# lightonai/next-plaid

Measured on AMD Instinct MI355X. Metric: queries/sec + p50 latency, k=10, 10M-doc x 300-tok x d128 PLAID index, 1/2/4/8 GPU, higher is better.
Workload: dtype f32 (split-bf16 hi/lo MFMA on the residual term of MaxSim, f32-class accuracy)

## Files before the change

next-plaid_amd/csrc/np_index.hip:

```cpp
#include "np_internal.h"

#include <hipcub/hipcub.hpp>

#include <algorithm>
#include <memory>
#include <thread>
#include <math.h>
#include <stdio.h>
#include <time.h>
#include <stdlib.h>
#include <string.h>

namespace np {

int DevBuf::reserve(size_t bytes) {
  if (bytes <= cap) return NP_OK;
  if (p) (void)hipFree(p);
  p = nullptr;
  cap = 0;
  size_t want = bytes + (bytes >> 3) + 256;
  hipError_t e = hipMalloc(&p, want);
  if (e != hipSuccess) {
    p = nullptr;
    set_error("hipMalloc(%zu bytes) failed: %s", want, hipGetErrorString(e));
// ... 29 lines not shown
  if (o->n_contexts <= 0) o->n_contexts = 2;
  if (o->n_contexts > 16) o->n_contexts = 16;
  if (o->max_batch <= 0) o->max_batch = 64;
  if (o->max_query_tokens <= 0) o->max_query_tokens = 64;
  return NP_OK;
}

bool set_tuning(Tuning* t, const std::string& n, int value) {
  auto clamp = [](int v, int lo, int hi) { return std::min(std::max(v, lo), hi); };
  if (n == "s4_mode") t->s4_mode = clamp(value, 0, 8);
  else if (n == "s4_minb") t->s4_minb = std::max(value, 1);
  else if (n == "s4_nbx") t->s4_nbx = clamp(value, 8, 512);
  else if (n == "s4_swz") t->s4_swz = value != 0;
  else if (n == "s4_filter") t->s4_filter = value != 0;
  else if (n == "s4_hot") t->s4_hot = clamp(value, 0, 500);
  else if (n == "s4_planes") t->s4_planes = value != 0;
  else if (n == "s4_pexp") t->s4_pexp = clamp(value, 5, 40);
  else if (n == "s4_lpd") t->s4_lpd = value == 2 ? 2 : 4;
  else if (n == "s4_qm") t->s4_qm = value != 0;
  else if (n == "s4_pnbx") t->s4_pnbx = clamp(value, 8, 512);
  else if (n == "s3_slices") t->s3_slices = value != 0;
  else if (n == "s4_warm") t->s4_warm = clamp(value, 0, 1000);
  else if (n == "ub_ncut") t->ub_ncut = clamp(value, 1, 512);
  else if (n == "s3_bisect") t->s3_bisect = clamp(value, 0, 1);
  else if (n == "s3_gain") t->s3_gain = clamp(value, 0, 2);
  else if (n == "s3_gain_mult") t->s3_gain_mult = clamp(value, 1, 16);
  else if (n == "s3_gain_direct") t->s3_gain_direct = clamp(value, 0, 64);
  else if (n == "s4_hot_auto") t->s4_hot_auto = clamp(value, 0, 0x7fffffff);
  else if (n == "ub_nt") t->ub_nt = value < 0 || value > 2 ? 0 : value;
  else if (n == "ub_steal") t->ub_steal = value < 1 ? 1 : value;
  else if (n == "ub_nbx") t->ub_nbx = clamp(value, 8, 256);
  else if (n == "ub_direct") t->ub_direct = clamp(value, 0, 16);
#ifdef NP_DIAGNOSTICS
  else if (n == "s4_probe") t->s4_probe = clamp(value, 0, 7);
#endif
  else if (n == "ub_static") t->ub_static = value != 0;
  else if (n == "hot_static") t->hot_static = value != 0;
  else if (n == "s6_xcd") t->s6_xcd = value != 0;
  else if (n == "s6_tiles") t->s6_tiles = value != 0;
  else if (n == "s6_lds") t->s6_lds = clamp(value, 0, 2);
  else if (n == "gemm_cpw") t->gemm_cpw = value == 2 ? 2 : 1;
  else if (n == "s1_split") t->s1_split = value != 0;
  else if (n == "exact_rowmax") t->exact_rowmax = value != 0;
  else return false;
  return true;
}

void read_tuning_env(Tuning* t) {
  static const char* const knobs[][2] = {
      {"NP_S4_MODE", "s4_mode"}, {"NP_S4_MINB", "s4_minb"}, {"NP_S4_NBX", "s4_nbx"}, {"NP_S4_SWZ", "s4_swz"},
      {"NP_S4_FILTER", "s4_filter"}, {"NP_S4_HOT", "s4_hot"}, {"NP_S4_PLANES", "s4_planes"}, {"NP_S4_PEXP", "s4_pexp"}, {"NP_S4_LPD", "s4_lpd"}, {"NP_S4_QM", "s4_qm"}, {"NP_S4_PNBX", "s4_pnbx"}, {"NP_S4_WARM", "s4_warm"}, {"NP_UB_NCUT", "ub_ncut"}, {"NP_S3_BISECT", "s3_bisect"}, {"NP_S3_GAIN", "s3_gain"}, {"NP_S3_GAIN_MULT", "s3_gain_mult"}, {"NP_S3_GAIN_DIRECT", "s3_gain_direct"}, {"NP_S4_HOT_AUTO", "s4_hot_auto"}, {"NP_S3_SLICES", "s3_slices"}, {"NP_UB_NT", "ub_nt"},
      {"NP_UB_STEAL", "ub_steal"}, {"NP_UB_NBX", "ub_nbx"}, {"NP_UB_DIRECT", "ub_direct"}, {"NP_UB_STATIC", "ub_static"}, {"NP_HOT_STATIC", "hot_static"}, {"NP_S6_XCD", "s6_xcd"}, {"NP_S6_TILES", "s6_tiles"}, {"NP_S6_LDS", "s6_lds"}, {"NP_GEMM_CPW", "gemm_cpw"}, {"NP_S1_SPLIT", "s1_split"},
      {"NP_EXACT_ROWMAX", "exact_rowmax"}};
  for (const auto& k : knobs) {
    const char* e = getenv(k[0]);
    if (e && *e) (void)set_tuning(t, k[1], atoi(e));
  }
#ifdef NP_DIAGNOSTICS
  if (const char* e = getenv("NP_S4_PROBE")) (void)set_tuning(t, "s4_probe", atoi(e));
#endif
}

static void default_workspace(DeviceIndex* ix) {
  ix->ws_auto = ix->opts.workspace_bytes <= 0;
  ix->ws_budget = ix->opts.workspace_bytes;
  ix->ws_budget_open = ix->opts.workspace_bytes;
  if (!ix->ws_auto) return;
  size_t free_b = 0, total_b = 0;
  int64_t ws = (int64_t)8 << 30;
  if (hipMemGetInfo(&free_b, &total_b) == hipSuccess) {
    const int64_t share = ((int64_t)free_b - ((int64_t)4 << 30)) / std::max(ix->opts.n_contexts, 1);
    ws = std::min<int64_t>((int64_t)16 << 30, std::max<int64_t>((int64_t)2 << 30, share));
  }
  ix->opts.workspace_bytes = ws;
// ... 1512 lines not shown
```

next-plaid_amd/csrc/np_internal.h:

```cpp
#pragma once
#include <hip/hip_runtime.h>
#include <stdint.h>
#include <algorithm>
#include <atomic>
#include <mutex>
#include <condition_variable>
#include <string>
#include <vector>
#include "../../include/nextplaid_hip.h"

namespace np {

struct CodeArr {
  const void* p;
  int wide;
  __device__ __forceinline__ uint32_t operator[](int64_t i) const {
    return wide ? static_cast<const uint32_t*>(p)[i] : (uint32_t)static_cast<const uint16_t*>(p)[i];
  }
};

void set_error(const char* fmt, ...) __attribute__((format(printf, 1, 2)));
const char* last_error();
void clear_error();

// ... 105 lines not shown
struct DevBuf {
  void* p = nullptr;
  size_t cap = 0;
  int reserve(size_t bytes);
  void release();
  template <class T> T* as() const { return (T*)p; }
};

struct Workspace;

struct Context {
  hipStream_t stream = nullptr;
  hipEvent_t ev[10] = {};
  Workspace* ws = nullptr;
  bool busy = false;
  uint64_t last_use = 0;
};

struct Tuning {
  int s4_mode = 4;
  int s4_minb = 8;
  int s4_nbx = 128;
  int s4_swz = 1;
  int s3_bisect = 1;
  int s3_slices = 1;
  int s3_gain = 1;
  int s3_gain_mult = 3;
  int s3_gain_direct = 16;
  int s4_filter = 1;
  int s4_hot = 60;
  int s4_hot_auto = 200000;
  int s4_planes = 1;
  int s4_lpd = 2;
  int s4_pnbx = 96;
  int s4_qm = 1;
  int s4_pexp = 15;
  int s4_warm = 0;
  int ub_ncut = 96;
  int ub_direct = 8;
  int hot_static = 1;
  int ub_static = 0;
  int s4_probe = 0;
  int ub_nbx = 96;
  int ub_steal = 16384;
  int ub_nt = 2;
  int s6_xcd = 1;
// ... 103 lines not shown
```

next-plaid_amd/csrc/np_kernels.h:

```cpp
#pragma once
#include <hip/hip_runtime.h>
#include <stdint.h>

namespace np {

typedef float f32x16 __attribute__((ext_vector_type(16)));
typedef __bf16 bf16x8 __attribute__((ext_vector_type(8)));

#define NP_NEG_INF (-__builtin_huge_valf())
#define NP_MAX_QT 8

__device__ __forceinline__ uint32_t okey(float x) {
  uint32_t b = __float_as_uint(x);
  uint32_t k = (b & 0x80000000u) ? ~b : (b | 0x80000000u);
  return ((b & 0x7F800000u) == 0x7F800000u) ? 0u : k;
}
__device__ __forceinline__ float unkey(uint32_t k) {
  uint32_t b = (k & 0x80000000u) ? (k ^ 0x80000000u) : ~k;
  return __uint_as_float(b);
}
__device__ __forceinline__ bool finitef(float x) { return (__float_as_uint(x) & 0x7F800000u) != 0x7F800000u; }
__device__ __forceinline__ float readlane_f(float v, int lane) {
  return __int_as_float(__builtin_amdgcn_readlane(__float_as_int(v), lane));
}
// ... 400 lines not shown
  }
}

struct ProbeP {
  const float* QCT;
  const uint32_t* gmax;
  const int32_t* qoff;
  int64_t K, KP;
  int LQP;
  int nprobe;
  const int32_t* nprobe_dev;
  const uint32_t* elig;
  const int32_t* n_elig;
  int has_thr;
  float thr;
  int lds_gm;
  int64_t slab;
  uint32_t* cellbits;
  uint32_t* tauq;
  uint32_t* cells_tmp;
  uint32_t* cells;
  int32_t* n_cells;
  Counters* ctr;
};

#define NP_PROBE_CAPG 64

template <class Pred>
__device__ __forceinline__ uint32_t wave_count(int nslots, const uint32_t (&keys)[32], Pred&& pred) {
  uint32_t mine = 0;
#pragma unroll
  for (int j = 0; j < 32; ++j) mine += (j < nslots && pred(keys[j])) ? 1u : 0u;
  uint32_t cnt = 0;
#pragma unroll
  for (int b = 0; b < 6; ++b) cnt += (uint32_t)__popcll(__ballot((mine >> b) & 1u)) << b;
  return cnt;
}

__device__ __forceinline__ void wave_select_mark(int nslots, uint32_t n_probe, const uint32_t (&keys)[32],
                                                 uint32_t& tau, uint32_t& rem) {
  uint32_t prefix = 0;
  for (int bit = 31; bit >= 0; --bit) {
    const uint32_t trial = prefix | (1u << bit);
    if (wave_count(nslots, keys, [&](uint32_t k) { return k >= trial; }) >= n_probe) prefix = trial;
  }
  const uint32_t gt = wave_count(nslots, keys, [&](uint32_t k) { return k > prefix; });
  tau = prefix;
  rem = n_probe > gt ? n_probe - gt : 0u;
}

template <int QW>
__global__ void __launch_bounds__(256) probe_mark_kernel(ProbeP p) {
  __shared__ uint32_t hist[256 * QW];
  __shared__ uint32_t part[256];
  __shared__ uint32_t s_prefix[QW], s_rem[QW], s_taug[QW], s_gcnt[QW];
  __shared__ uint32_t s_glist[QW * NP_PROBE_CAPG];
  extern __shared__ uint32_t s_gm[];
  constexpr int NR = 256 / QW;
  const bool lds_gm = p.lds_gm != 0;
  const int b = blockIdx.y, qc = blockIdx.x, tid = threadIdx.x, q = tid % QW, r = tid / QW;
  const int wave = tid >> 6, lane = tid & 63;
  const int Lq = p.qoff[b + 1] - p.qoff[b];
  const int64_t G = p.KP >> 5;
  const int LQP = p.LQP;
  const float* QCT = p.QCT + (int64_t)b * p.KP * LQP;
  const uint32_t* gm = p.gmax + (int64_t)b * G * LQP;
  uint32_t* bits = p.cellbits + (int64_t)b * G;
  const int64_t pool = p.elig ? (int64_t)*p.n_elig : p.K;
  const int64_t eff = p.nprobe_dev ? (int64_t)*p.nprobe_dev : (int64_t)p.nprobe;
  const uint32_t n_probe = (uint32_t)min(eff, pool);
  const bool take_all = pool <= (int64_t)n_probe;
  uint32_t* tauq = p.tauq + (int64_t)b * LQP;

  if (n_probe > 0 && take_all && Lq > 0) {
    if (qc != 0) return;
    for (int64_t w = tid; w < G; w += 256) {
      uint32_t m = p.elig ? p.elig[w] : 0xFFFFFFFFu;
      const int64_t c0 = w * 32;
      if (c0 + 32 > p.K) m &= (c0 >= p.K) ? 0u : ((1u << (p.K - c0)) - 1u);
      if (m) atomicOr(&bits[w], m);
    }
  } else if (n_probe > 0) {
    {
      if (qc * QW >= Lq) return;
      const int qq = qc * QW + q;
      const bool qvalid = qq < Lq;
      const bool use_groups = G > (int64_t)n_probe;
      if (lds_gm) {
        for (int64_t g0 = r; g0 < G; g0 += 16 * NR) {
          uint32_t kv[16];
#pragma unroll
          for (int u = 0; u < 16; ++u) kv[u] = (qvalid && g0 + NR * u < G) ? gm[(g0 + NR * u) * LQP + qq] : 0u;
#pragma unroll
          for (int u = 0; u < 16; ++u)
            if (g0 + NR * u < G) s_gm[(g0 + NR * u) * QW + q] = kv[u];
        }
        __syncthreads();
      }
      auto each_group = [&](auto&& cb) {
        if (!qvalid) return;
        if (lds_gm) {
          for (int64_t g = r; g < G; g += NR) cb(g, s_gm[g * QW + q]);
        } else {
          for (int64_t g = r; g < G; g += 8 * NR) {
            uint32_t kv[8];
#pragma unroll
            for (int u = 0; u < 8; ++u) kv[u] = (g + NR * u < G) ? gm[(g + NR * u) * LQP + qq] : 0u;
#pragma unroll
            for (int u = 0; u < 8; ++u)
              if (g + NR * u < G) cb(g + NR * u, kv[u]);
          }
        }
      };
      if (use_groups) {
        radix_select<QW>([&](auto&& cb) { each_group([&](int64_t, uint32_t key) { cb(key); }); }, n_probe, hist, part,
                         s_prefix, s_rem, tid);
        if (r == 0) s_taug[q] = s_prefix[q];
      } else if (r == 0) {
        s_taug[q] = 0;
      }
// ... 462 lines not shown
  int c = 0;
  for (int k = 0; k < NP_CHUNK_WORDS / 256; ++k) {
    const int64_t w = (int64_t)ch * NP_CHUNK_WORDS + k * 256 + threadIdx.x;
    if (w < NW) c += __popc(bits[w]);
  }
#pragma unroll
  for (int o = 32; o > 0; o >>= 1) c += __shfl_xor(c, o);
  if ((threadIdx.x & 63) == 0) atomicAdd(&s_cnt, c);
  __syncthreads();
  if (threadIdx.x == 0) chunk_counts[(int64_t)b * nchunks + ch] = s_cnt;
}

struct RoundPlan {
  int32_t* n_cand;
  int64_t* cand_base;
  int32_t* round_of;
  int32_t* round_tab;
  int32_t* order;
};

__global__ void __launch_bounds__(256) plan_rounds_kernel(const int32_t* __restrict__ chunk_counts, int nchunks, int B,
                                                          int64_t pool, int max_rounds, RoundPlan rp, Counters* ctr,
                                                          const int32_t* __restrict__ n_direct = nullptr ) {
  __shared__ int s_n[256];
  const int tid = threadIdx.x, lane = tid & 63, wave = tid >> 6;
  for (int b = wave; b < B; b += 4) {
    int c = 0;
    if (n_direct) c = lane == 0 ? n_direct[b] : 0;
    else
    for (int j = lane; j < nchunks; j += 64) c += chunk_counts[(int64_t)b * nchunks + j];
#pragma unroll
    for (int o = 32; o > 0; o >>= 1) c += __shfl_xor(c, o);
    if (lane == 0) s_n[b] = c;
  }
  __syncthreads();
  if (tid == 0) {
    int64_t cur = 0;
    unsigned long long total = 0;
    int r = 0;
    for (int i = 0; i < 2 * max_rounds; ++i) rp.round_tab[i] = 0;
    rp.round_tab[0] = 0;
    for (int b = 0; b < B; ++b) {
      const int n = s_n[b];
      if (cur + n > pool && r + 1 < max_rounds) {
        rp.round_tab[2 * r + 1] = b;
        ++r;
        rp.round_tab[2 * r] = b;
        cur = 0;
      }
      rp.n_cand[b] = (cur + n > pool) ? (int)max((int64_t)0, pool - cur) : n;
      rp.cand_base[b] = cur;
      rp.round_of[b] = r;
      cur += rp.n_cand[b];
      total += (unsigned long long)rp.n_cand[b];
    }
    rp.round_tab[2 * r + 1] = B;
    rp.round_tab[2 * max_rounds] = r + 1;
    if (!n_direct) atomicAdd(&ctr->n_candidates, total);
    atomicMax(&ctr->n_rounds, (unsigned long long)(r + 1));
  }
  __syncthreads();
  for (int b = tid; b < B; b += 256) {
    const int r = rp.round_of[b], rb = rp.round_tab[2 * r], re = rp.round_tab[2 * r + 1];
    const int n = rp.n_cand[b];
    int rank = 0;
    for (int j = rb; j < re; ++j) {
      const int nj = rp.n_cand[j];
      rank += (nj > n || (nj == n && j < b)) ? 1 : 0;
    }
    rp.order[rb + rank] = b;
  }
}

template <class Steal>
__device__ __forceinline__ int xcd_next_query(int32_t* slots, int32_t* ticket, int x, int step, int B,
                                              const int32_t* order, int rb, int re, Steal&& steal) {
  if (step > B) return -3;
  int32_t* slot = slots + (int64_t)x * (B + 1) + step;
  int v = __hip_atomic_load(slot, __ATOMIC_RELAXED, __HIP_MEMORY_SCOPE_AGENT);
  if (v == -1 && atomicCAS(slot, -1, -2) == -1) {
    const int t = atomicAdd(ticket, 1) + 1;
    v = (t < re - rb) ? order[rb + t] : steal();
    __hip_atomic_store(slot, v, __ATOMIC_RELAXED, __HIP_MEMORY_SCOPE_AGENT);
    return v;
  }
  while (v == -1 || v == -2) {
    __builtin_amdgcn_s_sleep(4);
    v = __hip_atomic_load(slot, __ATOMIC_RELAXED, __HIP_MEMORY_SCOPE_AGENT);
  }
  return v;
}

// ... 1404 lines not shown
    ndoc += __shfl_xor(ndoc, o);
  }
  __shared__ unsigned long long s_cnt[3];
  __syncthreads();
  if (tid == 0) s_cnt[0] = s_cnt[1] = s_cnt[2] = 0;
  __syncthreads();
  if (lane == 0 && toks) {
    atomicAdd(&s_cnt[0], toks);
    atomicAdd(&s_cnt[1], ucnt);
    atomicAdd(&s_cnt[2], ndoc);
  }
  __syncthreads();
  if (tid == 0 && s_cnt[0] && ctr) {
    if (count_tokens) {
      atomicAdd(&ctr->n_cand_tokens, s_cnt[0]);
      atomicAdd(&ctr->n_cand_dcodes, s_cnt[1]);
    } else {
      atomicAdd(&ctr->n_level2, s_cnt[2]);
    }
    atomicAdd(&ctr->n_cand_codes, s_cnt[1]);
  }
}

__global__ void __launch_bounds__(256) ub_thr_kernel(const uint32_t* __restrict__ hist, int hshift, int slack, int n_sel,
                                                     const int32_t* __restrict__ n_cand, RoundPlan rp, int round,
                                                     const uint32_t* __restrict__ qflag, uint32_t* __restrict__ thr) {
  __shared__ uint32_t s_part[256];
  constexpr int BPT = NP_UB_BINS / 256;
  const int b = blockIdx.x, tid = threadIdx.x;
  if (rp.round_of[b] != round) return;
  if (qflag[b] != 0 || n_cand[b] <= n_sel) {
    if (tid == 0) thr[b] = 0;
    return;
  }
  const uint32_t* hb = hist + (int64_t)b * NP_UB_BINS;
  const int top = (255 - tid) * BPT;
  uint32_t mine = 0;
#pragma unroll
  for (int k4 = 0; k4 < BPT / 4; ++k4) {
    const uint4 v = *reinterpret_cast<const uint4*>(hb + top + 4 * k4);
    mine += v.x + v.y + v.z + v.w;
  }
  s_part[tid] = mine;
  __syncthreads();
  if (tid == 0) {
    uint32_t cum = 0;
    int t = 0;
    for (; t < 255; ++t) {
      if (cum + s_part[t] >= (uint32_t)n_sel) break;
      cum += s_part[t];
    }
    int bin = (255 - t) * BPT + BPT - 1;
    for (; bin > (255 - t) * BPT; --bin) {
      if (cum + hb[bin] >= (uint32_t)n_sel) break;
      cum += hb[bin];
    }
    thr[b] = (uint32_t)max(0, bin - ((slack + (1 << hshift) - 1) >> hshift));
  }
}

struct CutP {
  const uint4* src;
  const int32_t* n_src_a;
  const int32_t* n_src_b;
  const uint16_t* U;
  const uint32_t* lo;
  const uint32_t* hi;
  int zero_mode;
  const uint4* all_src;
  const int32_t* n_all;
  uint4* dst;
  const int32_t* dst_begin;
  int32_t* n_dst;
  int hshift;
  Counters* ctr;
};

__global__ void __launch_bounds__(256) ub_cut_kernel(CutP p, RoundPlan rp, int round) {
  __shared__ int s_wcnt[4], s_base;
  __shared__ unsigned long long s_cnt[2];
  const int b = blockIdx.y, tid = threadIdx.x, lane = tid & 63, wave = tid >> 6;
  if (rp.round_of[b] != round) return;
  const uint32_t lo = p.lo[b], hi = p.hi ? p.hi[b] : 0xFFFFFFFFu;
  const bool all = lo == 0;
  if (all && p.zero_mode == 1) return;
  const uint4* src = all ? p.all_src : p.src;
  const int64_t n = all ? (int64_t)p.n_all[b] : (int64_t)p.n_src_a[b] + (p.n_src_b ? p.n_src_b[b] : 0);
  const int64_t pbase = rp.cand_base[b];
  const int64_t dbase = pbase + (p.dst_begin ? p.dst_begin[b] : 0);
  if (tid == 0) s_cnt[0] = s_cnt[1] = 0;
  unsigned long long toks = 0, ucnt = 0;
  constexpr int PT = 8;
  for (int64_t i0 = (int64_t)blockIdx.x * (256 * PT); i0 < n; i0 += (int64_t)gridDim.x * (256 * PT)) {
    bool keep[PT];
    unsigned long long bal[PT];
    int wtot = 0;
#pragma unroll
    for (int k = 0; k < PT; ++k) {
      const int64_t i = i0 + k * 256 + tid;
      bool kp = i < n;
      if (kp && !all) {
        const uint32_t bin = min((uint32_t)p.U[pbase + i] >> p.hshift, (uint32_t)(NP_UB_BINS - 1));
        kp = bin >= lo && bin < hi;
      }
      keep[k] = kp;
      bal[k] = __ballot(kp);
// ... 2515 lines not shown
```

next-plaid_amd/csrc/np_search.hip:

```cpp
#include "np_internal.h"
#include "np_kernels.h"

#include <algorithm>
#include <array>
#include <cmath>
#include <stdlib.h>
#include <string.h>
#include <type_traits>
#include <utility>

namespace np {

struct Workspace {
  DevBuf q, qoff, Qt, Qb, Qbl, QCT, gmax, tauq, cellbits, cells_tmp, cells, n_cells, docbits, chunk_counts, cand, cand_meta, approx, n_cand,
      cand_base, round_of, round_tab, QCU, qinv, qflag, ub, ub_hist, ub_thr, ub_cursor, q_order, xcd_slots, surv_meta, n_surv, n_list2, sel_keys, sel_doc, nsel, exact, out_ids, out_scores, out_keys, out_counts, ctr, subset,
      subset_bits, elig, misc, cut, cmaxu, chist, ub2, ub_hist2, ub_thr2, list_meta, n_l1, n_l2, qpad, planes, levels, hotbits,
      gain, gsmall, ghist, s0_meta, s0_u, gacc, gdeep;
  void* h_pin = nullptr;
  size_t h_pin_cap = 0;
  unsigned long long* h_gain = nullptr;
  uint64_t h_gain_key = 0;
  hipEvent_t done = nullptr;
  bool done_valid = false;
  static constexpr int NBUF = 66;
  std::array<DevBuf*, NBUF> all_bufs() {
    return {&q, &qoff, &Qt, &Qb, &Qbl, &QCT, &gmax, &tauq, &cellbits, &cells_tmp, &cells, &n_cells, &docbits, &chunk_counts, &cand, &cand_meta, &approx, &n_cand, &cand_base, &round_of, &round_tab, &QCU, &qinv, &qflag, &ub, &ub_hist, &ub_thr, &ub_cursor, &q_order, &xcd_slots, &surv_meta, &n_surv, &n_list2, &sel_keys, &sel_doc, &nsel, &exact, &out_ids, &out_scores, &out_keys, &out_counts, &ctr, &subset, &subset_bits, &elig, &misc, &cut, &cmaxu, &chist, &ub2, &ub_hist2, &ub_thr2, &list_meta, &n_l1, &n_l2, &qpad, &planes, &levels, &hotbits, &gain, &gsmall, &ghist, &s0_meta, &s0_u, &gacc, &gdeep};
  }
  void release_all() {
    for (DevBuf* b : all_bufs()) b->release();
    if (h_pin) (void)hipHostFree(h_pin);
    h_pin = nullptr;
    h_pin_cap = 0;
    if (h_gain) (void)hipHostFree(h_gain);
    h_gain = nullptr;
    if (done) (void)hipEventDestroy(done);
    done = nullptr;
  }
  size_t total_bytes() {
    size_t t = 0;
    for (DevBuf* b : all_bufs()) t += b->cap;
    return t;
  }
  unsigned probe_tick = 0;
  size_t pool_bytes() const {
    return cand.cap + cand_meta.cap + approx.cap + ub.cap + surv_meta.cap + ub2.cap + list_meta.cap;
  }
  void release_pool() {
    DevBuf* pool[] = {&cand, &cand_meta, &approx, &ub, &surv_meta, &ub2, &list_meta};
    for (DevBuf* b : pool) b->release();
// ... 127 lines not shown
    return NP_ERR_INVALID_ARGUMENT;
  }
  return NP_OK;
}

constexpr int NP_POOL_ENTRY = 60;
struct WsPlan {
  int S = 1;
  int64_t pool = 1;
  int max_rounds = 1;
};

static int64_t per_query_bytes(const DeviceIndex* ix, int LQP, int n_sel, int top_k) {
  const int64_t KP = ix->KP, G = KP / 32, NW = (ix->n_docs + 31) / 32;
  const int64_t nchunks = (NW + NP_CHUNK_WORDS - 1) / NP_CHUNK_WORDS;
  return KP * LQP * 6
         + KP + 1024
         + KP * 6 + G * 4 + NP_UB_BINS * 8
         + (ix->d_ivf_split.get() ? (int64_t)ix->n_ranges * NP_GAIN_RANGE : 0)
         + NP_UB_BINS * 8
         + G * LQP * 4 + G * 4
         + KP * 8
         + (int64_t)LQP * 4
         + std::max<int64_t>(NW, 1) * 4
         + std::max<int64_t>(nchunks, 1) * 4
         + (int64_t)ix->dim * LQP * 8
         + (int64_t)std::max(n_sel, 1) * 16 + (int64_t)std::max(top_k, 1) * 20 + 64;
}

static WsPlan plan_workspace(const DeviceIndex* ix, int B, int LQP, const np_search_params* prm, int64_t probed_cells = 0) {
  WsPlan w;
  const int64_t budget = ix->ws_budget.load(std::memory_order_relaxed);
  const int64_t pq = std::max<int64_t>(per_query_bytes(ix, LQP, n_sel_of(prm), prm->top_k), 1);
  const int64_t nd = std::max<int64_t>(ix->n_docs, 1);
  const int cap = (int)std::min<int64_t>(std::min<int64_t>(ix->opts.max_batch, NP_S4_MAXB), std::max(B, 1));
  int64_t S = std::min<int64_t>(cap, std::max<int64_t>(1, (budget * 3 / 4) / pq));
  while (S > 1 && S * pq + 2 * nd * NP_POOL_ENTRY > budget) --S;
  w.S = (int)S;
  int64_t worst_q = nd;
  if (probed_cells > 0 && !ix->ivf_top_prefix.empty())
    worst_q = std::max<int64_t>(1, std::min(nd, ix->ivf_top_prefix[(size_t)std::min<int64_t>(probed_cells, ix->K)]));
  const int64_t worst = S * worst_q;
  int64_t pool = (budget - S * pq) / NP_POOL_ENTRY;
  pool = std::min(worst, std::max(pool, std::min<int64_t>(2, S) * worst_q));
  w.pool = std::max<int64_t>(pool, 1);
  w.max_rounds = (worst <= w.pool) ? 1 : (int)std::min<int64_t>(S, worst / (w.pool - worst_q + 1) + 1);
// ... 356 lines not shown
  if (!ix->gain_run.load(std::memory_order_relaxed)) ix->gain_skip.store(3, std::memory_order_relaxed);
  return true;
}

static void settle_zeroth_level(const DeviceIndex* ix, Workspace& w, const CallState* cs, PassPlan& p) {
  p.gain_path = p.gain_possible && (ix->tune.s3_gain != 1 || gain_level_runs(ix, w, cs, p.B, p.LQP));
  p.gain_deep = p.gain_path && p.deep_wanted;
  if (p.gain_path && cs->prm.has_threshold && !p.gain_deep) p.gain_path = false;
}

static int reserve_pass(const DeviceIndex* ix, const CallState* cs, const PassPlan& p, Workspace& w) {
  const size_t B = (size_t)p.B, KP = (size_t)p.KP, G = (size_t)p.G, LQP = (size_t)p.LQP, dim = (size_t)ix->dim;
  const size_t pool = (size_t)p.pool, RB = (size_t)p.RB;
  const size_t nsel1 = (size_t)std::max(cs->n_sel, 1), topk1 = (size_t)std::max(cs->prm.top_k, 1);
  const size_t nw1 = (size_t)std::max<int64_t>(p.NW, 1);
  if (ix->ldim != ix->dim) NP_TRY(w.qpad.reserve((size_t)std::max<int64_t>(p.rows, 1) * dim * 4));
  NP_TRY(w.Qt.reserve(B * dim * LQP * 4));
  NP_TRY(w.Qb.reserve(B * dim * LQP * 2));
  NP_TRY(w.Qbl.reserve(B * dim * LQP * 2));
  NP_TRY(w.QCT.reserve(B * KP * LQP * 4));
  NP_TRY(w.gmax.reserve(B * G * LQP * 4));
  NP_TRY(w.cellbits.reserve(B * G * 4));
  NP_TRY(w.tauq.reserve(B * LQP * 4));
  NP_TRY(w.cells_tmp.reserve(B * KP * 4));
  NP_TRY(w.cells.reserve(B * KP * 4));
  NP_TRY(w.n_cells.reserve(B * 4));
  NP_TRY(w.docbits.reserve(B * nw1 * 4));
  NP_TRY(w.chunk_counts.reserve(B * (size_t)std::max(p.nchunks, 1) * 4));
  NP_TRY(w.cand.reserve(pool * 4));
  NP_TRY(w.cand_meta.reserve(pool * 16));
  NP_TRY(w.approx.reserve(pool * 4));
  NP_TRY(w.n_cand.reserve(B * 4));
  NP_TRY(w.cand_base.reserve(B * 8));
  NP_TRY(w.round_of.reserve(B * 4));
  NP_TRY(w.round_tab.reserve((size_t)(2 * p.max_rounds + 1) * 4));
  NP_TRY(w.q_order.reserve(B * 4));
  NP_TRY(w.n_list2.reserve(B * 4));
  NP_TRY(w.qinv.reserve(B * 4));
  NP_TRY(w.qflag.reserve(B * 4));
  if (p.use_filter) {
    NP_TRY(w.QCU.reserve(B * KP * RB));
    NP_TRY(w.ub.reserve(pool * 2));
    NP_TRY(w.ub_hist.reserve(B * NP_UB_BINS * 4));
    NP_TRY(w.surv_meta.reserve(pool * 16));
    NP_TRY(w.n_surv.reserve(B * 4));
    NP_TRY(w.ub_thr.reserve(B * 4));
// ... 164 lines not shown
  const np_search_params& prm = cs->prm;
  ProbeP pp;
  pp.QCT = w.QCT.as<float>();
  pp.gmax = w.gmax.as<uint32_t>();
  pp.qoff = d_qoff;
  pp.K = ix->K;
  pp.KP = p.KP;
  pp.LQP = p.LQP;
  pp.nprobe = prm.n_ivf_probe;
  pp.nprobe_dev = p.use_elig ? w.misc.as<int32_t>() + 1 : nullptr;
  pp.elig = p.use_elig ? (cs->elig_global ? cs->elig_global : w.elig.as<uint32_t>()) : nullptr;
  pp.n_elig = p.use_elig ? w.misc.as<int32_t>() : nullptr;
  pp.has_thr = prm.has_threshold;
  pp.thr = prm.centroid_score_threshold;
  pp.slab = p.batched ? (int64_t)prm.centroid_batch_size : 0;
  pp.cellbits = w.cellbits.as<uint32_t>();
  pp.tauq = w.tauq.as<uint32_t>();
  pp.cells_tmp = w.cells_tmp.as<uint32_t>();
  pp.cells = w.cells.as<uint32_t>();
  pp.n_cells = w.n_cells.as<int32_t>();
  pp.ctr = w.ctr.as<Counters>();
  const size_t gm_lds = (size_t)(p.KP / 32) * 4 * 4;
  pp.lds_gm = gm_lds <= 32 * 1024 ? 1 : 0;
  auto probe = [&](const ProbeP& pr) {
    if (pr.lds_gm) probe_mark_kernel<4><<<dim3((unsigned)(p.LQP / 4), B), 256, gm_lds, st>>>(pr);
    else probe_mark_kernel<8><<<dim3((unsigned)(p.LQP / 8), B), 256, 0, st>>>(pr);
    probe_finish_kernel<<<dim3(NP_PROBE_NF, B), 256, 0, st>>>(pr);
  };
  probe(pp);
  if (!p.gain_deep) return;
  const GDeep gd(w.gdeep.p, p);
  ProbeP p2 = pp;
  p2.nprobe = p.gain_depth;
  p2.has_thr = 0;
  p2.cellbits = gd.marks;
  p2.tauq = gd.tauq;
  p2.n_cells = gd.n_cells;
  p2.cells = gd.cells;
  p2.ctr = nullptr;
  probe(p2);
  if (prm.has_threshold)
    cells_to_bits_kernel<<<B, 256, 0, st>>>(w.cells.as<uint32_t>(), w.n_cells.as<int32_t>(), p.KP, gd.kept);
}

RoundPlan Pass::round_plan() const {
  RoundPlan rp;
  rp.n_cand = w.n_cand.as<int32_t>();
  rp.cand_base = w.cand_base.as<int64_t>();
  rp.round_of = w.round_of.as<int32_t>();
  rp.round_tab = w.round_tab.as<int32_t>();
  rp.order = w.q_order.as<int32_t>();
  return rp;
}

int Pass::ub_bounds(const RoundPlan& rpx, int r, int max_rounds, int32_t* sl, uint32_t* cur, const uint4* meta,
                    const int32_t* begin, const int32_t* count, const int32_t* n_all, uint16_t* U, uint32_t* hist,
                    int count_tokens, int direct_wpq, bool floor_rows) const {
// ... 183 lines not shown
    }
  } else if (ix->T > 0) {
    if (matvec) {
      launch_matvec(st, ix, w, d_q, d_qoff, B, w.cand_meta.as<uint4>(), w.n_cand.as<int32_t>(), rp, r);
      count_work_kernel<<<dim3(32, (unsigned)B), 256, 0, st>>>(w.cand_meta.as<uint4>(), w.n_cand.as<int32_t>(), rp, r,
                                                               w.ctr.as<Counters>());
    } else {
      launch_approx(st, ix, w, d_qoff, B, p.LQP, w.cand_meta.as<uint4>(), w.n_cand.as<int32_t>(), rp, r, p.max_rounds,
                    w.ctr.as<Counters>());
    }
  }
  if (cs->timed && r == 0) NP_HIP(hipEventRecord(cs->ctx->ev[4], st));
  if (cs->n_sel > 0) {
    sp.round = r;
    select_kernel<<<B, 1024, (size_t)cs->NSELP * 8, st>>>(sp);
  }
  return NP_OK;
}

int Pass::single_level_cut(int r, const RoundPlan& rp) const {
  const int B = p.B;
  NP_TRY(ub_bounds(rp, r, p.max_rounds, slots((size_t)r * 3), cursor(0), w.cand_meta.as<uint4>(), nullptr, w.n_cand.as<int32_t>(),
                   w.n_cand.as<int32_t>(), w.ub.as<uint16_t>(), w.ub_hist.as<uint32_t>(), 1, 0, false));
  ub_thr_kernel<<<B, 256, 0, st>>>(w.ub_hist.as<uint32_t>(), p.hshift, p.slack, cs->n_sel, w.n_cand.as<int32_t>(), rp, r,
                                   w.qflag.as<uint32_t>(), w.ub_thr.as<uint32_t>());
  CutP cp{};
  cp.hshift = p.hshift;
  cp.all_src = w.cand_meta.as<uint4>();
  cp.n_all = w.n_cand.as<int32_t>();
  cp.src = w.cand_meta.as<uint4>();
  cp.n_src_a = w.n_cand.as<int32_t>();
  cp.U = w.ub.as<uint16_t>();
  cp.lo = w.ub_thr.as<uint32_t>();
  cp.zero_mode = 0;
  cp.dst = w.surv_meta.as<uint4>();
  cp.n_dst = w.n_surv.as<int32_t>();
  cp.ctr = w.ctr.as<Counters>();
  ub_cut_kernel<<<dim3(n_cut(), B), 256, 0, st>>>(cp, rp, r);
  return NP_OK;
}

int Pass::two_level_cut(int r, const RoundPlan& rp) const {
  const int B = p.B;
  const unsigned ncut = n_cut();
  auto ub = [&](int lvl, const int32_t* begin, const int32_t* count, int direct_wpq, bool floor_rows) {
    return ub_bounds(rp, r, p.max_rounds, slots((size_t)r * 3 + lvl), cursor(lvl), w.list_meta.as<uint4>(), begin, count,
                     w.n_cand.as<int32_t>(), w.ub2.as<uint16_t>(), w.ub_hist2.as<uint32_t>(), 0, direct_wpq, floor_rows);
  };
  CutP cp{};
  cp.hshift = p.hshift;
  cp.all_src = w.cand_meta.as<uint4>();
  cp.n_all = w.n_cand.as<int32_t>();
  if (cs->timed && r == 0) NP_HIP(hipEventRecord(cs->ctx->ev[8], st));
  NP_TRY(hot_level(r, rp));
  if (cs->timed && r == 0) {
    NP_HIP(hipEventRecord(cs->ctx->ev[9], st));
    cs->hot_timed = true;
  }
  ub_thr_kernel<<<B, 256, 0, st>>>(w.ub_hist.as<uint32_t>(), p.hshift, 0, cs->n_sel, w.n_cand.as<int32_t>(), rp, r,
                                   w.qflag.as<uint32_t>(), w.ub_thr.as<uint32_t>());
  cp.src = w.cand_meta.as<uint4>();
  cp.n_src_a = w.n_cand.as<int32_t>();
  cp.U = w.ub.as<uint16_t>();
  cp.lo = w.ub_thr.as<uint32_t>();
  cp.zero_mode = 1;
  cp.dst = w.list_meta.as<uint4>();
  cp.n_dst = w.n_l1.as<int32_t>();
  ub_cut_kernel<<<dim3(ncut, B), 256, 0, st>>>(cp, rp, r);
  NP_TRY(ub(1, nullptr, w.n_l1.as<int32_t>(), ix->tune.ub_direct, false));
  ub_thr_kernel<<<B, 256, 0, st>>>(w.ub_hist2.as<uint32_t>(), p.hshift, p.slack, cs->n_sel, w.n_cand.as<int32_t>(), rp, r,
                                   w.qflag.as<uint32_t>(), w.ub_thr2.as<uint32_t>());
  cp.lo = w.ub_thr2.as<uint32_t>();
  cp.hi = w.ub_thr.as<uint32_t>();
  cp.dst_begin = w.n_l1.as<int32_t>();
  cp.n_dst = w.n_l2.as<int32_t>();
  ub_cut_kernel<<<dim3(ncut, B), 256, 0, st>>>(cp, rp, r);
  NP_TRY(ub(2, w.n_l1.as<int32_t>(), w.n_l2.as<int32_t>(), 0, true));
  ub_thr_kernel<<<B, 256, 0, st>>>(w.ub_hist2.as<uint32_t>(), p.hshift, p.slack, cs->n_sel, w.n_cand.as<int32_t>(), rp, r,
                                   w.qflag.as<uint32_t>(), w.ub_thr2.as<uint32_t>());
  cp.src = w.list_meta.as<uint4>();
  cp.n_src_a = w.n_l1.as<int32_t>();
  cp.n_src_b = w.n_l2.as<int32_t>();
  cp.U = w.ub2.as<uint16_t>();
  cp.lo = w.ub_thr2.as<uint32_t>();
  cp.hi = nullptr;
  cp.zero_mode = 0;
  cp.dst = w.surv_meta.as<uint4>();
  cp.dst_begin = nullptr;
  cp.n_dst = w.n_surv.as<int32_t>();
  cp.ctr = w.ctr.as<Counters>();
  ub_cut_kernel<<<dim3(ncut, B), 256, 0, st>>>(cp, rp, r);
  return NP_OK;
}

int Pass::hot_level(int r, const RoundPlan& rp) const {
  const int B = p.B;
  const int64_t KP = p.KP;
  const int old_cap = ix->code_wide ? 64 : 128;
  const int plpd = (ix->ublock_stride > old_cap || ix->tune.s4_lpd == 4) ? 4 : 2;
  const unsigned pnbx = (unsigned)ix->tune.s4_pnbx;
  return with_codes(ix->code_wide, [&](auto ct) -> int {
    using CT = decltype(ct);
// ... 856 lines not shown
```

Measured before the change: 20290.

## Add threshold-first probe list, fuse UB threshold into cut, parallelize round planning

Three separate changes. A new probe_thr_kernel first lists the centroids whose max score clears the query threshold, so the probe marking kernel can rank only those listed cells and fall back to the full group scan when the list overflows. Separately, the ub_thr_kernel launches are removed: each ub_cut_kernel block now computes the histogram threshold itself through a parallel wave scan, and one block writes it out. plan_rounds_kernel is also rewritten to build its round table and ordering from shared-memory arrays in parallel instead of serially through global memory. Together these aim to cut kernel launches and serial work, at the cost of repeating the threshold scan in every cut block and extra complexity in the probe path.

```diff
diff --git a/next-plaid_amd/csrc/np_index.hip b/next-plaid_amd/csrc/np_index.hip
--- a/next-plaid_amd/csrc/np_index.hip
+++ b/next-plaid_amd/csrc/np_index.hip
@@ -75,6 +75,7 @@
   else if (n == "s3_slices") t->s3_slices = value != 0;
   else if (n == "s4_warm") t->s4_warm = clamp(value, 0, 1000);
   else if (n == "ub_ncut") t->ub_ncut = clamp(value, 1, 512);
+  else if (n == "s2_thr_first") t->s2_thr_first = value != 0;
   else if (n == "s3_bisect") t->s3_bisect = clamp(value, 0, 1);
   else if (n == "s3_gain") t->s3_gain = clamp(value, 0, 2);
   else if (n == "s3_gain_mult") t->s3_gain_mult = clamp(value, 1, 16);
@@ -102,7 +103,7 @@
 void read_tuning_env(Tuning* t) {
   static const char* const knobs[][2] = {
       {"NP_S4_MODE", "s4_mode"}, {"NP_S4_MINB", "s4_minb"}, {"NP_S4_NBX", "s4_nbx"}, {"NP_S4_SWZ", "s4_swz"},
-      {"NP_S4_FILTER", "s4_filter"}, {"NP_S4_HOT", "s4_hot"}, {"NP_S4_PLANES", "s4_planes"}, {"NP_S4_PEXP", "s4_pexp"}, {"NP_S4_LPD", "s4_lpd"}, {"NP_S4_QM", "s4_qm"}, {"NP_S4_PNBX", "s4_pnbx"}, {"NP_S4_WARM", "s4_warm"}, {"NP_UB_NCUT", "ub_ncut"}, {"NP_S3_BISECT", "s3_bisect"}, {"NP_S3_GAIN", "s3_gain"}, {"NP_S3_GAIN_MULT", "s3_gain_mult"}, {"NP_S3_GAIN_DIRECT", "s3_gain_direct"}, {"NP_S4_HOT_AUTO", "s4_hot_auto"}, {"NP_S3_SLICES", "s3_slices"}, {"NP_UB_NT", "ub_nt"},
+      {"NP_S4_FILTER", "s4_filter"}, {"NP_S4_HOT", "s4_hot"}, {"NP_S4_PLANES", "s4_planes"}, {"NP_S4_PEXP", "s4_pexp"}, {"NP_S4_LPD", "s4_lpd"}, {"NP_S4_QM", "s4_qm"}, {"NP_S4_PNBX", "s4_pnbx"}, {"NP_S4_WARM", "s4_warm"}, {"NP_UB_NCUT", "ub_ncut"}, {"NP_S3_BISECT", "s3_bisect"}, {"NP_S2_THR_FIRST", "s2_thr_first"}, {"NP_S3_GAIN", "s3_gain"}, {"NP_S3_GAIN_MULT", "s3_gain_mult"}, {"NP_S3_GAIN_DIRECT", "s3_gain_direct"}, {"NP_S4_HOT_AUTO", "s4_hot_auto"}, {"NP_S3_SLICES", "s3_slices"}, {"NP_UB_NT", "ub_nt"},
       {"NP_UB_STEAL", "ub_steal"}, {"NP_UB_NBX", "ub_nbx"}, {"NP_UB_DIRECT", "ub_direct"}, {"NP_UB_STATIC", "ub_static"}, {"NP_HOT_STATIC", "hot_static"}, {"NP_S6_XCD", "s6_xcd"}, {"NP_S6_TILES", "s6_tiles"}, {"NP_S6_LDS", "s6_lds"}, {"NP_GEMM_CPW", "gemm_cpw"}, {"NP_S1_SPLIT", "s1_split"},
       {"NP_EXACT_ROWMAX", "exact_rowmax"}};
   for (const auto& k : knobs) {
diff --git a/next-plaid_amd/csrc/np_internal.h b/next-plaid_amd/csrc/np_internal.h
--- a/next-plaid_amd/csrc/np_internal.h
+++ b/next-plaid_amd/csrc/np_internal.h
@@ -151,6 +151,7 @@
   int s4_minb = 8;
   int s4_nbx = 128;
   int s4_swz = 1;
+  int s2_thr_first = 1;
   int s3_bisect = 1;
   int s3_slices = 1;
   int s3_gain = 1;
diff --git a/next-plaid_amd/csrc/np_kernels.h b/next-plaid_amd/csrc/np_kernels.h
--- a/next-plaid_amd/csrc/np_kernels.h
+++ b/next-plaid_amd/csrc/np_kernels.h
@@ -446,7 +446,83 @@
   uint32_t* cells;
   int32_t* n_cells;
   Counters* ctr;
+  uint32_t* thr_list;
+  const uint32_t* qflag;
 };
+
+#define NP_PROBE_THR_CAP 64
+#define NP_PROBE_THR_OVF 0xFFFFFFFFu
+
+__global__ void __launch_bounds__(1024) probe_thr_kernel(ProbeP p) {
+  __shared__ uint32_t s_ng, s_nl;
+  __shared__ uint32_t s_g[NP_PROBE_THR_CAP], s_l[NP_PROBE_THR_CAP];
+  extern __shared__ uint32_t s_seen[];
+  const int b = blockIdx.x, tid = threadIdx.x;
+  const int Lq = p.qoff[b + 1] - p.qoff[b];
+  const int64_t G = p.KP >> 5;
+  const int LQP = p.LQP, L4 = LQP >> 2;
+  const float* QCT = p.QCT + (int64_t)b * p.KP * LQP;
+  const uint4* gm4 = reinterpret_cast<const uint4*>(p.gmax + (int64_t)b * G * LQP);
+  uint32_t* out = p.thr_list + (int64_t)b * (1 + NP_PROBE_THR_CAP);
+  if (p.qflag[b] != 0 || Lq <= 0) {
+    if (tid == 0) out[0] = NP_PROBE_THR_OVF;
+    return;
+  }
+  if (tid == 0) s_ng = s_nl = 0;
+  for (int64_t w = tid; w < (G + 31) / 32; w += 1024) s_seen[w] = 0;
+  __syncthreads();
+  const float thr = p.thr;
+  const int64_t n4 = G * L4;
+  for (int64_t i0 = tid; i0 < n4; i0 += 4 * 1024) {
+    uint4 v[4];
+#pragma unroll
+    for (int u = 0; u < 4; ++u) v[u] = (i0 + u * 1024 < n4) ? gm4[i0 + u * 1024] : make_uint4(0, 0, 0, 0);
+#pragma unroll
+    for (int u = 0; u < 4; ++u) {
+      const int64_t i = i0 + u * 1024;
+      if (i >= n4) break;
+      const int64_t g = i / L4;
+      const int q0 = (int)(i - g * L4) * 4;
+      const bool pass = (q0 < Lq && unkey(v[u].x) >= thr) || (q0 + 1 < Lq && unkey(v[u].y) >= thr) ||
+                        (q0 + 2 < Lq && unkey(v[u].z) >= thr) || (q0 + 3 < Lq && unkey(v[u].w) >= thr);
+      if (pass) {
+        const uint32_t bit = 1u << (g & 31);
+        if (!(atomicOr(&s_seen[g >> 5], bit) & bit)) {
+          const uint32_t pos = atomicAdd(&s_ng, 1u);
+          if (pos < NP_PROBE_THR_CAP) s_g[pos] = (uint32_t)g;
+        }
+      }
+    }
+  }
+  __syncthreads();
+  const uint32_t ng = s_ng;
+  if (ng > NP_PROBE_THR_CAP) {
+    if (tid == 0) out[0] = NP_PROBE_THR_OVF;
+    return;
+  }
+  for (uint32_t e = tid; e < ng * 32; e += 1024) {
+    const int64_t c = (int64_t)s_g[e >> 5] * 32 + (e & 31);
+    if (c >= p.K) continue;
+    const float4* row4 = reinterpret_cast<const float4*>(QCT + c * LQP);
+    uint32_t km = 0;
+    for (int q4 = 0; 4 * q4 < Lq; ++q4) {
+      const float4 v = row4[q4];
+      km = max(km, okey(v.x));
+      if (4 * q4 + 1 < Lq) km = max(km, okey(v.y));
+      if (4 * q4 + 2 < Lq) km = max(km, okey(v.z));
+      if (4 * q4 + 3 < Lq) km = max(km, okey(v.w));
+    }
+    const float mx = km != 0 ? unkey(km) : QCT[c * LQP + Lq - 1];
+    if (mx >= thr) {
+      const uint32_t pos = atomicAdd(&s_nl, 1u);
+      if (pos < NP_PROBE_THR_CAP) s_l[pos] = (uint32_t)c;
+    }
+  }
+  __syncthreads();
+  const uint32_t nl = s_nl;
+  if (nl <= NP_PROBE_THR_CAP && (uint32_t)tid < nl) out[1 + tid] = s_l[tid];
+  if (tid == 0) out[0] = nl <= NP_PROBE_THR_CAP ? nl : NP_PROBE_THR_OVF;
+}
 
 #define NP_PROBE_CAPG 64
 
@@ -479,6 +555,7 @@
   __shared__ uint32_t part[256];
   __shared__ uint32_t s_prefix[QW], s_rem[QW], s_taug[QW], s_gcnt[QW];
   __shared__ uint32_t s_glist[QW * NP_PROBE_CAPG];
+  __shared__ int s_legacy;
   extern __shared__ uint32_t s_gm[];
   constexpr int NR = 256 / QW;
   const bool lds_gm = p.lds_gm != 0;
@@ -509,6 +586,12 @@
       if (qc * QW >= Lq) return;
       const int qq = qc * QW + q;
       const bool qvalid = qq < Lq;
+      const uint32_t* tlist = p.thr_list ? p.thr_list + (int64_t)b * (1 + NP_PROBE_THR_CAP) : nullptr;
+      const uint32_t nlist = tlist ? tlist[0] : NP_PROBE_THR_OVF;
+      if (nlist == 0) return;
+      const bool listed = nlist != NP_PROBE_THR_OVF;
+      if (tid == 0) s_legacy = 0;
+      if (!lds_gm) __syncthreads();
       const bool use_groups = G > (int64_t)n_probe;
       if (lds_gm) {
         for (int64_t g0 = r; g0 < G; g0 += 16 * NR) {
@@ -520,6 +603,62 @@
             if (g0 + NR * u < G) s_gm[(g0 + NR * u) * QW + q] = kv[u];
         }
         __syncthreads();
+      }
+      if (listed) {
+        const int nq = min(QW, Lq - qc * QW);
+        const uint32_t npairs = nlist * (uint32_t)nq;
+        uint32_t* glist = s_glist + wave * NP_PROBE_CAPG;
+        auto gkey = [&](int64_t g, int t) { return lds_gm ? s_gm[g * QW + t] : gm[g * LQP + qc * QW + t]; };
+        for (uint32_t base = 0; base < npairs; base += 256) {
+          const uint32_t mp = base + 4u * lane + wave;
+          uint32_t mc = 0, mk = 0;
+          if (mp < npairs) {
+            mc = tlist[1 + mp / nq];
+            mk = okey(QCT[(int64_t)mc * LQP + qc * QW + (int)(mp % nq)]);
+          }
+          for (int l = 0; l < 64; ++l) {
+            const uint32_t pr = base + 4u * l + wave;
+            if (pr >= npairs) break;
+            const uint32_t c = (uint32_t)__shfl((int)mc, l), k = (uint32_t)__shfl((int)mk, l);
+            const int t = (int)(pr % nq);
+            uint32_t above = 0;
+            for (int64_t g0 = 0; g0 < G && above < n_probe; g0 += 64) {
+              const int64_t g = g0 + lane;
+              above += (uint32_t)__popcll(__ballot(g < G && gkey(g, t) > k));
+            }
+            if (above >= n_probe) continue;
+            uint32_t ng = 0;
+            for (int64_t g0 = 0; g0 < G; g0 += 64) {
+              const int64_t g = g0 + lane;
+              const bool ge = g < G && gkey(g, t) >= k;
+              const unsigned long long bal = __ballot(ge);
+              const uint32_t pos = ng + (uint32_t)__popcll(bal & ((1ull << lane) - 1ull));
+              if (ge && pos < NP_PROBE_CAPG) glist[pos] = (uint32_t)g;
+              ng += (uint32_t)__popcll(bal);
+            }
+            if (ng > NP_PROBE_CAPG) {
+              if (lane == 0) s_legacy = 1;
+              continue;
+            }
+            __builtin_amdgcn_fence(__ATOMIC_RELEASE, "wavefront");
+            __builtin_amdgcn_wave_barrier();
+            const float* col = QCT + qc * QW + t;
+            uint32_t mine = 0;
+            for (uint32_t e = lane; e < ng * 32; e += 64) {
+              const int64_t c2 = (int64_t)glist[e >> 5] * 32 + (e & 31);
+              if (c2 < p.K) {
+                const uint32_t k2 = okey(col[c2 * LQP]);
+                mine += (k2 > k || (k2 == k && c2 < (int64_t)c)) ? 1u : 0u;
+              }
+            }
+#pragma unroll
+            for (int o = 32; o > 0; o >>= 1) mine += (uint32_t)__shfl_xor((int)mine, o);
+            if (mine < n_probe && lane == 0) atomicOr(&bits[c >> 5], 1u << (c & 31));
+            __builtin_amdgcn_wave_barrier();
+          }
+        }
+        __syncthreads();
+        if (!s_legacy) return;
       }
       auto each_group = [&](auto&& cb) {
         if (!qvalid) return;
@@ -1028,7 +1167,9 @@
 __global__ void __launch_bounds__(256) plan_rounds_kernel(const int32_t* __restrict__ chunk_counts, int nchunks, int B,
                                                           int64_t pool, int max_rounds, RoundPlan rp, Counters* ctr,
                                                           const int32_t* __restrict__ n_direct = nullptr ) {
-  __shared__ int s_n[256];
+  __shared__ int s_n[256], s_r[256];
+  __shared__ int64_t s_base[256];
+  __shared__ int s_nr;
   const int tid = threadIdx.x, lane = tid & 63, wave = tid >> 6;
   for (int b = wave; b < B; b += 4) {
     int c = 0;
@@ -1044,36 +1185,43 @@
     int64_t cur = 0;
     unsigned long long total = 0;
     int r = 0;
-    for (int i = 0; i < 2 * max_rounds; ++i) rp.round_tab[i] = 0;
-    rp.round_tab[0] = 0;
     for (int b = 0; b < B; ++b) {
       const int n = s_n[b];
       if (cur + n > pool && r + 1 < max_rounds) {
-        rp.round_tab[2 * r + 1] = b;
         ++r;
-        rp.round_tab[2 * r] = b;
         cur = 0;
       }
-      rp.n_cand[b] = (cur + n > pool) ? (int)max((int64_t)0, pool - cur) : n;
-      rp.cand_base[b] = cur;
-      rp.round_of[b] = r;
-      cur += rp.n_cand[b];
-      total += (unsigned long long)rp.n_cand[b];
-    }
-    rp.round_tab[2 * r + 1] = B;
+      const int nc = (cur + n > pool) ? (int)max((int64_t)0, pool - cur) : n;
+      s_n[b] = nc;
+      s_base[b] = cur;
+      s_r[b] = r;
+      cur += nc;
+      total += (unsigned long long)nc;
+    }
+    s_nr = r + 1;
     rp.round_tab[2 * max_rounds] = r + 1;
     if (!n_direct) atomicAdd(&ctr->n_candidates, total);
     atomicMax(&ctr->n_rounds, (unsigned long long)(r + 1));
   }
   __syncthreads();
+  const int nr = s_nr;
+  for (int i = tid; i < 2 * max_rounds; i += 256) {
+    const int k = i >> 1, upto = k + (i & 1);
+    int cnt = 0;
+    for (int j = 0; j < B; ++j) cnt += s_r[j] < upto ? 1 : 0;
+    rp.round_tab[i] = k < nr ? cnt : 0;
+  }
   for (int b = tid; b < B; b += 256) {
-    const int r = rp.round_of[b], rb = rp.round_tab[2 * r], re = rp.round_tab[2 * r + 1];
-    const int n = rp.n_cand[b];
-    int rank = 0;
-    for (int j = rb; j < re; ++j) {
-      const int nj = rp.n_cand[j];
-      rank += (nj > n || (nj == n && j < b)) ? 1 : 0;
-    }
+    const int r = s_r[b], n = s_n[b];
+    int rb = 0, rank = 0;
+    for (int j = 0; j < B; ++j) {
+      const int rj = s_r[j], nj = s_n[j];
+      rb += rj < r ? 1 : 0;
+      rank += (rj == r && (nj > n || (nj == n && j < b))) ? 1 : 0;
+    }
+    rp.n_cand[b] = n;
+    rp.cand_base[b] = s_base[b];
+    rp.round_of[b] = r;
     rp.order[rb + rank] = b;
   }
 }
@@ -2524,41 +2672,52 @@
   }
 }
 
+__device__ __forceinline__ uint32_t ub_thr_block(const uint32_t* __restrict__ hb , int hshift,
+                                                 int slack, int n_sel, int n_cand, uint32_t flag, uint32_t* s_w) {
+  constexpr int BPT = NP_UB_BINS / 256;
+  static_assert(BPT == 8, "two uint4 loads per thread");
+  if (flag != 0 || n_cand <= n_sel) return 0;
+  const int tid = threadIdx.x, lane = tid & 63, wave = tid >> 6;
+  const int top = (255 - tid) * BPT;
+  const uint4 v0 = *reinterpret_cast<const uint4*>(hb + top), v1 = *reinterpret_cast<const uint4*>(hb + top + 4);
+  const uint32_t h[BPT] = {v0.x, v0.y, v0.z, v0.w, v1.x, v1.y, v1.z, v1.w};
+  const uint32_t mine = v0.x + v0.y + v0.z + v0.w + v1.x + v1.y + v1.z + v1.w;
+  uint32_t incl = mine;
+#pragma unroll
+  for (int o = 1; o < 64; o <<= 1) {
+    const uint32_t v = (uint32_t)__shfl_up((int)incl, o);
+    if (lane >= o) incl += v;
+  }
+  __syncthreads();
+  if (lane == 63) s_w[wave] = incl;
+  __syncthreads();
+  for (int k = 0; k < wave; ++k) incl += s_w[k];
+  const uint32_t ns = (uint32_t)n_sel, excl = incl - mine;
+  const bool owner = tid < 255 ? (incl >= ns && (tid == 0 || excl < ns)) : excl < ns;
+  if (owner) {
+    uint32_t cum = excl;
+    int k = BPT - 1;
+#pragma unroll
+    for (int u = BPT - 1; u > 0; --u) {
+      if (k == u && cum + h[u] < ns) {
+        cum += h[u];
+        k = u - 1;
+      }
+    }
+    s_w[4] = (uint32_t)max(0, top + k - ((slack + (1 << hshift) - 1) >> hshift));
+  }
+  __syncthreads();
+  return s_w[4];
+}
+
 __global__ void __launch_bounds__(256) ub_thr_kernel(const uint32_t* __restrict__ hist, int hshift, int slack, int n_sel,
                                                      const int32_t* __restrict__ n_cand, RoundPlan rp, int round,
                                                      const uint32_t* __restrict__ qflag, uint32_t* __restrict__ thr) {
-  __shared__ uint32_t s_part[256];
-  constexpr int BPT = NP_UB_BINS / 256;
-  const int b = blockIdx.x, tid = threadIdx.x;
+  __shared__ uint32_t s_w[5];
+  const int b = blockIdx.x;
   if (rp.round_of[b] != round) return;
-  if (qflag[b] != 0 || n_cand[b] <= n_sel) {
-    if (tid == 0) thr[b] = 0;
-    return;
-  }
-  const uint32_t* hb = hist + (int64_t)b * NP_UB_BINS;
-  const int top = (255 - tid) * BPT;
-  uint32_t mine = 0;
-#pragma unroll
-  for (int k4 = 0; k4 < BPT / 4; ++k4) {
-    const uint4 v = *reinterpret_cast<const uint4*>(hb + top + 4 * k4);
-    mine += v.x + v.y + v.z + v.w;
-  }
-  s_part[tid] = mine;
-  __syncthreads();
-  if (tid == 0) {
-    uint32_t cum = 0;
-    int t = 0;
-    for (; t < 255; ++t) {
-      if (cum + s_part[t] >= (uint32_t)n_sel) break;
-      cum += s_part[t];
-    }
-    int bin = (255 - t) * BPT + BPT - 1;
-    for (; bin > (255 - t) * BPT; --bin) {
-      if (cum + hb[bin] >= (uint32_t)n_sel) break;
-      cum += hb[bin];
-    }
-    thr[b] = (uint32_t)max(0, bin - ((slack + (1 << hshift) - 1) >> hshift));
-  }
+  const uint32_t t = ub_thr_block(hist + (int64_t)b * NP_UB_BINS, hshift, slack, n_sel, n_cand[b], qflag[b], s_w);
+  if (threadIdx.x == 0) thr[b] = t;
 }
 
 struct CutP {
@@ -2566,7 +2725,10 @@
   const int32_t* n_src_a;
   const int32_t* n_src_b;
   const uint16_t* U;
-  const uint32_t* lo;
+  uint32_t* lo;
+  const uint32_t* hist;
+  int slack, n_sel;
+  const uint32_t* qflag;
   const uint32_t* hi;
   int zero_mode;
   const uint4* all_src;
@@ -2581,9 +2743,12 @@
 __global__ void __launch_bounds__(256) ub_cut_kernel(CutP p, RoundPlan rp, int round) {
   __shared__ int s_wcnt[4], s_base;
   __shared__ unsigned long long s_cnt[2];
+  __shared__ uint32_t s_w[5];
   const int b = blockIdx.y, tid = threadIdx.x, lane = tid & 63, wave = tid >> 6;
   if (rp.round_of[b] != round) return;
-  const uint32_t lo = p.lo[b], hi = p.hi ? p.hi[b] : 0xFFFFFFFFu;
+  const uint32_t lo = ub_thr_block(p.hist + (int64_t)b * NP_UB_BINS, p.hshift, p.slack, p.n_sel, p.n_all[b], p.qflag[b], s_w);
+  const uint32_t hi = p.hi ? p.hi[b] : 0xFFFFFFFFu;
+  if (blockIdx.x == 0 && tid == 0) p.lo[b] = lo;
   const bool all = lo == 0;
   if (all && p.zero_mode == 1) return;
   const uint4* src = all ? p.all_src : p.src;
diff --git a/next-plaid_amd/csrc/np_search.hip b/next-plaid_amd/csrc/np_search.hip
--- a/next-plaid_amd/csrc/np_search.hip
+++ b/next-plaid_amd/csrc/np_search.hip
@@ -15,16 +15,17 @@
   DevBuf q, qoff, Qt, Qb, Qbl, QCT, gmax, tauq, cellbits, cells_tmp, cells, n_cells, docbits, chunk_counts, cand, cand_meta, approx, n_cand,
       cand_base, round_of, round_tab, QCU, qinv, qflag, ub, ub_hist, ub_thr, ub_cursor, q_order, xcd_slots, surv_meta, n_surv, n_list2, sel_keys, sel_doc, nsel, exact, out_ids, out_scores, out_keys, out_counts, ctr, subset,
       subset_bits, elig, misc, cut, cmaxu, chist, ub2, ub_hist2, ub_thr2, list_meta, n_l1, n_l2, qpad, planes, levels, hotbits,
-      gain, gsmall, ghist, s0_meta, s0_u, gacc, gdeep;
+      gain, gsmall, ghist, s0_meta, s0_u, gacc, gdeep,
+      thr_list;
   void* h_pin = nullptr;
   size_t h_pin_cap = 0;
   unsigned long long* h_gain = nullptr;
   uint64_t h_gain_key = 0;
   hipEvent_t done = nullptr;
   bool done_valid = false;
-  static constexpr int NBUF = 66;
+  static constexpr int NBUF = 67;
   std::array<DevBuf*, NBUF> all_bufs() {
-    return {&q, &qoff, &Qt, &Qb, &Qbl, &QCT, &gmax, &tauq, &cellbits, &cells_tmp, &cells, &n_cells, &docbits, &chunk_counts, &cand, &cand_meta, &approx, &n_cand, &cand_base, &round_of, &round_tab, &QCU, &qinv, &qflag, &ub, &ub_hist, &ub_thr, &ub_cursor, &q_order, &xcd_slots, &surv_meta, &n_surv, &n_list2, &sel_keys, &sel_doc, &nsel, &exact, &out_ids, &out_scores, &out_keys, &out_counts, &ctr, &subset, &subset_bits, &elig, &misc, &cut, &cmaxu, &chist, &ub2, &ub_hist2, &ub_thr2, &list_meta, &n_l1, &n_l2, &qpad, &planes, &levels, &hotbits, &gain, &gsmall, &ghist, &s0_meta, &s0_u, &gacc, &gdeep};
+    return {&q, &qoff, &Qt, &Qb, &Qbl, &QCT, &gmax, &tauq, &cellbits, &cells_tmp, &cells, &n_cells, &docbits, &chunk_counts, &cand, &cand_meta, &approx, &n_cand, &cand_base, &round_of, &round_tab, &QCU, &qinv, &qflag, &ub, &ub_hist, &ub_thr, &ub_cursor, &q_order, &xcd_slots, &surv_meta, &n_surv, &n_list2, &sel_keys, &sel_doc, &nsel, &exact, &out_ids, &out_scores, &out_keys, &out_counts, &ctr, &subset, &subset_bits, &elig, &misc, &cut, &cmaxu, &chist, &ub2, &ub_hist2, &ub_thr2, &list_meta, &n_l1, &n_l2, &qpad, &planes, &levels, &hotbits, &gain, &gsmall, &ghist, &s0_meta, &s0_u, &gacc, &gdeep, &thr_list};
   }
   void release_all() {
     for (DevBuf* b : all_bufs()) b->release();
@@ -198,6 +199,7 @@
          + G * LQP * 4 + G * 4
          + KP * 8
          + (int64_t)LQP * 4
+         + (1 + NP_PROBE_THR_CAP) * 4
          + std::max<int64_t>(NW, 1) * 4
          + std::max<int64_t>(nchunks, 1) * 4
          + (int64_t)ix->dim * LQP * 8
@@ -600,6 +602,7 @@
   NP_TRY(w.gmax.reserve(B * G * LQP * 4));
   NP_TRY(w.cellbits.reserve(B * G * 4));
   NP_TRY(w.tauq.reserve(B * LQP * 4));
+  NP_TRY(w.thr_list.reserve(B * (1 + NP_PROBE_THR_CAP) * 4));
   NP_TRY(w.cells_tmp.reserve(B * KP * 4));
   NP_TRY(w.cells.reserve(B * KP * 4));
   NP_TRY(w.n_cells.reserve(B * 4));
@@ -810,6 +813,10 @@
   pp.ctr = w.ctr.as<Counters>();
   const size_t gm_lds = (size_t)(p.KP / 32) * 4 * 4;
   pp.lds_gm = gm_lds <= 32 * 1024 ? 1 : 0;
+  const bool thr_first = ix->tune.s2_thr_first && prm.has_threshold && !p.batched && !p.use_elig && (!p.gain_path || p.gain_deep);
+  pp.thr_list = thr_first ? w.thr_list.as<uint32_t>() : nullptr;
+  pp.qflag = w.qflag.as<uint32_t>();
+  if (thr_first) probe_thr_kernel<<<B, 1024, (size_t)((p.G + 31) / 32) * 4, st>>>(pp);
   auto probe = [&](const ProbeP& pr) {
     if (pr.lds_gm) probe_mark_kernel<4><<<dim3((unsigned)(p.LQP / 4), B), 256, gm_lds, st>>>(pr);
     else probe_mark_kernel<8><<<dim3((unsigned)(p.LQP / 8), B), 256, 0, st>>>(pr);
@@ -821,6 +828,7 @@
   ProbeP p2 = pp;
   p2.nprobe = p.gain_depth;
   p2.has_thr = 0;
+  p2.thr_list = nullptr;
   p2.cellbits = gd.marks;
   p2.tauq = gd.tauq;
   p2.n_cells = gd.n_cells;
@@ -1050,10 +1058,12 @@
   const int B = p.B;
   NP_TRY(ub_bounds(rp, r, p.max_rounds, slots((size_t)r * 3), cursor(0), w.cand_meta.as<uint4>(), nullptr, w.n_cand.as<int32_t>(),
                    w.n_cand.as<int32_t>(), w.ub.as<uint16_t>(), w.ub_hist.as<uint32_t>(), 1, 0, false));
-  ub_thr_kernel<<<B, 256, 0, st>>>(w.ub_hist.as<uint32_t>(), p.hshift, p.slack, cs->n_sel, w.n_cand.as<int32_t>(), rp, r,
-                                   w.qflag.as<uint32_t>(), w.ub_thr.as<uint32_t>());
   CutP cp{};
   cp.hshift = p.hshift;
+  cp.hist = w.ub_hist.as<uint32_t>();
+  cp.slack = p.slack;
+  cp.n_sel = cs->n_sel;
+  cp.qflag = w.qflag.as<uint32_t>();
   cp.all_src = w.cand_meta.as<uint4>();
   cp.n_all = w.n_cand.as<int32_t>();
   cp.src = w.cand_meta.as<uint4>();
@@ -1077,6 +1087,8 @@
   };
   CutP cp{};
   cp.hshift = p.hshift;
+  cp.n_sel = cs->n_sel;
+  cp.qflag = w.qflag.as<uint32_t>();
   cp.all_src = w.cand_meta.as<uint4>();
   cp.n_all = w.n_cand.as<int32_t>();
   if (cs->timed && r == 0) NP_HIP(hipEventRecord(cs->ctx->ev[8], st));
@@ -1085,8 +1097,8 @@
     NP_HIP(hipEventRecord(cs->ctx->ev[9], st));
     cs->hot_timed = true;
   }
-  ub_thr_kernel<<<B, 256, 0, st>>>(w.ub_hist.as<uint32_t>(), p.hshift, 0, cs->n_sel, w.n_cand.as<int32_t>(), rp, r,
-                                   w.qflag.as<uint32_t>(), w.ub_thr.as<uint32_t>());
+  cp.hist = w.ub_hist.as<uint32_t>();
+  cp.slack = 0;
   cp.src = w.cand_meta.as<uint4>();
   cp.n_src_a = w.n_cand.as<int32_t>();
   cp.U = w.ub.as<uint16_t>();
@@ -1096,16 +1108,14 @@
   cp.n_dst = w.n_l1.as<int32_t>();
   ub_cut_kernel<<<dim3(ncut, B), 256, 0, st>>>(cp, rp, r);
   NP_TRY(ub(1, nullptr, w.n_l1.as<int32_t>(), ix->tune.ub_direct, false));
-  ub_thr_kernel<<<B, 256, 0, st>>>(w.ub_hist2.as<uint32_t>(), p.hshift, p.slack, cs->n_sel, w.n_cand.as<int32_t>(), rp, r,
-                                   w.qflag.as<uint32_t>(), w.ub_thr2.as<uint32_t>());
+  cp.hist = w.ub_hist2.as<uint32_t>();
+  cp.slack = p.slack;
   cp.lo = w.ub_thr2.as<uint32_t>();
   cp.hi = w.ub_thr.as<uint32_t>();
   cp.dst_begin = w.n_l1.as<int32_t>();
   cp.n_dst = w.n_l2.as<int32_t>();
   ub_cut_kernel<<<dim3(ncut, B), 256, 0, st>>>(cp, rp, r);
   NP_TRY(ub(2, w.n_l1.as<int32_t>(), w.n_l2.as<int32_t>(), 0, true));
-  ub_thr_kernel<<<B, 256, 0, st>>>(w.ub_hist2.as<uint32_t>(), p.hshift, p.slack, cs->n_sel, w.n_cand.as<int32_t>(), rp, r,
-                                   w.qflag.as<uint32_t>(), w.ub_thr2.as<uint32_t>());
   cp.src = w.list_meta.as<uint4>();
   cp.n_src_a = w.n_l1.as<int32_t>();
   cp.n_src_b = w.n_l2.as<int32_t>();
```

Result: no change. 20340, median of 3 (+0.2%).
